# bastienjacquet/CudaDepthMapIntegration

Hardware: AMD Instinct MI355X
Metric: Gvoxel-projections/s (higher is better)
Workload: dtype f64

## Files before the change

### cudadepthmapintegration_amd/capi.py

```python
from __future__ import annotations

import ctypes
import os
import sys
from typing import NamedTuple

import numpy as np

from . import build as _build
from .scene import GridDesc, RayPotential, Views

DMI_OK = 0
DMI_F32, DMI_F64 = 0, 1
DMI_DEPTH_AUTO, DMI_DEPTH_F32, DMI_DEPTH_F64 = 0, 1, 2
DMI_COMPONENTS_MIN_TRIANGLES, DMI_COMPONENTS_LARGEST = 0, 1

VARIANT_EXACT_DIVISION = 1
VARIANT_GENERAL_K = 2
VARIANT_FORCE_GENERAL = 16
VARIANT_NO_BRICK_CLASSES = 256
VARIANT_KEEP_BEHIND_ADDS = 1024
VARIANT_NO_INTERIOR = 2048
VARIANT_XCD_RUNS = 8192
VARIANT_ZMAJOR_SLOTS = 16384
VARIANT_PERSISTENT_ALWAYS = 32768
VARIANT_PERSISTENT_NEVER = 65536
VARIANT_NO_WINDOWS = 262144
VARIANT_WINDOWS_ALWAYS = 524288
VARIANT_COST_ORDER = 1048576
VARIANT_NO_COST_ORDER = 2097152
VARIANT_BRICK_CLASSES_ALWAYS = 131072
VARIANT_FIXED_TILE_SHAPE = 4096
VARIANT_SPATIAL_ORDER = 512
VARIANT_TILE_SHAPE = {"tk16_w5_g8_1x1": 0, "tk8_w6_g8_2x2": 32, "tk16_w5_g8_2x2": 64, "tk8_w6": 96, "tk8_w7_g8": 128, "tk16_w5_g4": 160,
                      "tk16_w6_g2": 192, "tk8_w6_g8_1x1": 224}


class GridDescC(ctypes.Structure):
    _fields_ = [("cell_dims", ctypes.c_int32 * 3), ("origin", ctypes.c_double * 3),
                ("spacing", ctypes.c_double * 3), ("grid_matrix", ctypes.c_double * 16)]


class RayPotentialC(ctypes.Structure):
    _fields_ = [("thickness", ctypes.c_double), ("rho", ctypes.c_double), ("eta", ctypes.c_double),
                ("delta", ctypes.c_double)]
# ... 77 lines not shown
DMI_PARTITION_VIEWS, DMI_PARTITION_Z_SLABS = 0, 1
DMI_EXCHANGE_ALL_REDUCE, DMI_EXCHANGE_REDUCE_SCATTER, DMI_EXCHANGE_PEER_COPY = 0, 1, 2
DMI_UNIQUE_ID_BYTES = 128
RENDER_VIEW_GROUP, RENDER_LANE_CAP = 16, 64

DMI_DECIMATE_MEAN, DMI_DECIMATE_QUADRIC = 0, 1
DECIMATE_PLACEMENTS = {"mean": DMI_DECIMATE_MEAN, "quadric": DMI_DECIMATE_QUADRIC}

ABI_SYMBOLS = [
    "dmi_default_options", "dmi_create", "dmi_destroy", "dmi_last_error", "dmi_add_views", "dmi_add_views_f32",
    "dmi_clear_views", "dmi_reset_grid", "dmi_upload_grid", "dmi_fuse", "dmi_fuse_range", "dmi_fuse_slab", "dmi_fuse_range_download", "dmi_synchronize",
    "dmi_download_grid_f64", "dmi_download_grid_f32", "dmi_download_hits", "dmi_grid_device_pointer",
    "dmi_get_brick_class_histogram", "dmi_get_timings", "dmi_get_info", "dmi_alloc_pinned", "dmi_free_pinned", "dmi_pcie_probe", "dmi_fp64_probe", "dmi_abi_version", "dmi_device_count",
    "dmi_color_mesh", "dmi_color_last_error", "dmi_cell_to_point", "dmi_download_point_data_f64",
    "dmi_point_data_device_pointer", "dmi_color_create", "dmi_color_destroy", "dmi_color_add_views",
    "dmi_color_clear_views", "dmi_color_process", "dmi_color_get_kernel_ms", "dmi_get_mixed_reason_histogram", "dmi_get_window_pair_count", "dmi_get_view_paths", "dmi_get_upload_kernel_ms", "dmi_sizeof_info", "dmi_sizeof_timings",
    "dmi_color_set_scratch_budget", "dmi_color_set_vertex_reorder", "dmi_color_add_views_with_depth", "dmi_color_set_depth_test",
    "dmi_iso_active_cells",
    "dmi_extract_isosurface", "dmi_download_isosurface", "dmi_get_isosurface_kernel_ms",
    "dmi_extract_isosurface_normals", "dmi_download_isosurface_normals",
    "dmi_filter_isosurface_components", "dmi_download_isosurface_regions", "dmi_get_isosurface_filter_kernel_ms",
    "dmi_get_isosurface_filter_pass_ms", "dmi_get_isosurface_filter_cas_retries",
    "dmi_smooth_isosurface", "dmi_get_isosurface_smooth_kernel_ms", "dmi_get_isosurface_smooth_pass_ms",
    "dmi_decimate_isosurface", "dmi_get_isosurface_decimate_kernel_ms", "dmi_get_isosurface_decimate_pass_ms",
    "dmi_color_process_isosurface", "dmi_download_isosurface_colors", "dmi_get_isosurface_color_kernel_ms",
    "dmi_filter_isosurface_support", "dmi_download_isosurface_support", "dmi_get_isosurface_support_kernel_ms",
    "dmi_get_isosurface_support_pass_ms", "dmi_decimate_isosurface_placed",
    "dmi_fill_isosurface_holes", "dmi_get_isosurface_holes_kernel_ms", "dmi_get_isosurface_holes_pass_ms",
    "dmi_color_render_depths", "dmi_color_render_isosurface_depths", "dmi_color_download_depths", "dmi_color_get_render_kernel_ms",
    "dmi_color_set_render_queue_capacity", "dmi_color_get_render_pass_ms", "dmi_color_get_render_queued_pairs",
    "dmi_filter_depth_consistency", "dmi_estimate_scene_bounds", "dmi_filter_depth_speckles", "dmi_fill_depth_holes",
# ... 111 lines not shown
        L.dmi_get_isosurface_holes_pass_ms.argtypes = [vp, dp]
    if hasattr(L, "dmi_filter_isosurface_support"):
        L.dmi_filter_isosurface_support.argtypes = [vp, i32, dbl, i32, ctypes.POINTER(ctypes.c_uint64), ctypes.POINTER(ctypes.c_uint64)]
        L.dmi_download_isosurface_support.argtypes = [vp, ctypes.POINTER(ctypes.c_int32)]
        L.dmi_get_isosurface_support_kernel_ms.argtypes = [vp, dp]
        L.dmi_get_isosurface_support_pass_ms.argtypes = [vp, dp]
    if hasattr(L, "dmi_set_point_smoothing"):
        L.dmi_point_smoothing_weights.argtypes = [dbl, dbl, ctypes.POINTER(i32), dp]
        L.dmi_set_point_smoothing.argtypes = [vp, dp, dbl]
        L.dmi_get_point_smoothing.argtypes = [vp, dp, dp]
        L.dmi_get_point_smoothing_kernel_ms.argtypes = [vp, dp]
    L.dmi_get_brick_class_histogram.argtypes = [vp, ctypes.POINTER(ctypes.c_uint64)]
    L.dmi_get_mixed_reason_histogram.argtypes = [vp, ctypes.POINTER(ctypes.c_uint64)]
    if hasattr(L, "dmi_get_window_pair_count"):
        L.dmi_get_window_pair_count.argtypes = [vp, ctypes.POINTER(ctypes.c_uint64)]
    if hasattr(L, "dmi_get_view_paths"):
        L.dmi_get_view_paths.argtypes = [vp, ctypes.POINTER(ctypes.c_uint64)]
    if hasattr(L, "dmi_get_upload_kernel_ms"):
        L.dmi_get_upload_kernel_ms.argtypes = [vp, dp, dp]
    for name in ("dmi_sizeof_info", "dmi_sizeof_timings"):
        if hasattr(L, name):
            getattr(L, name).restype = ctypes.c_size_t
    L.dmi_get_timings.argtypes = [vp, ctypes.POINTER(TimingsC)]
    L.dmi_get_info.argtypes = [vp, ctypes.POINTER(InfoC)]
    L.dmi_alloc_pinned.argtypes = [ctypes.c_size_t, ctypes.POINTER(vp)]
    L.dmi_free_pinned.argtypes = [vp]
    L.dmi_pcie_probe.argtypes = [i32, ctypes.c_size_t, dp, dp]
    L.dmi_fp64_probe.argtypes = [i32, ctypes.c_double, dp]
    u8p = ctypes.POINTER(ctypes.c_uint8)
    L.dmi_color_mesh.argtypes = [dp, ctypes.c_int64, u8p, dp, dp, i32, i32, i32, i32, u8p, u8p, ctypes.POINTER(ctypes.c_int32)]
# ... 498 lines not shown

    def mixed_reason_histogram(self) -> dict:
        h = (ctypes.c_uint64 * 8)()
        self._check(self._lib.dmi_get_mixed_reason_histogram(self._h, h))
        names = ["unspecified", "degenerate", "camera_plane", "image_border", "nan_depth", "sentinel_and_depth", "near_surface",
                 "free_or_no_depth"]
        return {n: int(h[i]) for i, n in enumerate(names)}

    def window_pair_count(self) -> int:
        n = ctypes.c_uint64(0)
        if not hasattr(self._lib, "dmi_get_window_pair_count"):
            return 0
        self._check(self._lib.dmi_get_window_pair_count(self._h, ctypes.byref(n)))
        return int(n.value)

    def upload_kernel_ms(self) -> tuple:
        if not hasattr(self._lib, "dmi_get_upload_kernel_ms"):
            return (0.0, 0.0)
        a, b = ctypes.c_double(0), ctypes.c_double(0)
        self._check(self._lib.dmi_get_upload_kernel_ms(self._h, ctypes.byref(a), ctypes.byref(b)))
        return (float(a.value), float(b.value))

    def timings(self) -> TimingsC:
        t = TimingsC()
        self._check(self._lib.dmi_get_timings(self._h, ctypes.byref(t)))
        return t

    def info(self) -> InfoC:
        i = InfoC()
        self._check(self._lib.dmi_get_info(self._h, ctypes.byref(i)))
# ... 1241 lines not shown
```

### cudadepthmapintegration_amd/csrc/dmi_capi_fuse.hip

```cpp
#include "dmi_context.h"

#include <algorithm>
#include <cmath>
#include <cstdlib>
#include <cstring>

using dmi::drain_events;
using dmi::EventPair;
using dmi::fail;
using dmi::flush_zero_fill;
using dmi::FuseArgs;
using dmi::FuseConfig;
using dmi::guarded;
using dmi::MapRec;
using dmi::TileArgs;
using dmi::TileMapRec;

namespace {

static_assert(dmi::kRecordBytes[dmi::REC_MAP] == sizeof(MapRec) && dmi::kRecordBytes[dmi::REC_TILE_MAP] == sizeof(TileMapRec) &&
              dmi::kRecordBytes[dmi::REC_WIN] == sizeof(dmi::WinRec) && dmi::kRecordBytes[dmi::REC_FOOT] == sizeof(dmi::FootRec) &&
              dmi::kRecordBytes[dmi::REC_HITS] == sizeof(unsigned long long), "the record tables' rule has the records' sizes");
int sync_maps(dmi_context *ctx) {
  dmi_context::Views &v = ctx->views;
// ... 151 lines not shown
  const int rc = slot_permutation(ctx, t.super_x, t.super_y, t.super_z, (cfg.variant & dmi::VAR_ZMAJOR_SLOTS) != 0, &t.sb_perm);
  if (rc != DMI_OK) return rc;
  t.xcd_run_wg = 32 * std::max(1, t.super_x * t.super_y);
  if (((int64_t)t.super_x * t.super_y * t.super_z * 32 + 16 * (int64_t)t.xcd_run_wg + 64) > (int64_t)0x7fffffff)
    return fail(ctx, DMI_ERR_INVALID_ARGUMENT, "dmi_fuse: grid too large for one launch");
  t.depth_bytes = (int32_t)((int64_t)a.W * a.H * (ctx->views.depth_f64 ? 8 : 4));
  t.kz0 = a.kz0;
  t.ox = a.ox; t.oy = a.oy; t.oz = a.oz; t.sx = a.sx; t.sy = a.sy; t.sz = a.sz;
  std::memcpy(t.g, a.g, sizeof(t.g));
  t.thick = a.thick; t.delta = a.delta; t.rho_pos = a.rho_pos; t.rho_neg = a.rho_neg;
  t.slope = a.slope; t.free_space = a.free_space;
  t.tile_maps = ctx->views.tile_maps.as<TileMapRec>();
  t.grid = a.grid; t.voxel_hits = a.voxel_hits; t.map_hits = a.map_hits;
  t.rotated = dmi::grid_axis_aligned(ctx->grid) ? 0 : 1;
  t.flags = ((cfg.variant & dmi::VAR_NO_INTERIOR) ? dmi::TILE_FLAG_NO_INTERIOR : 0) |
            ((cfg.variant & dmi::VAR_XCD_RUNS) ? dmi::TILE_FLAG_XCD_RUNS : 0);
  t.maps = ctx->views.maps.as<MapRec>();
  t.wbricks_x = (a.nx + 7) / 8;
  t.wbricks_y = (a.ny + 7) / 8;
  return DMI_OK;
}

int cz_table(dmi_context *ctx, const FuseArgs &a, TileArgs *t) {
  const size_t table_doubles = std::max<size_t>(ctx->views.h_maps.size(), 4) * (size_t)t->kpad;
  const size_t need = table_doubles + (size_t)dmi::kFreeSumsMax + 1;
  const int rc = dmi::ensure_idle_buffer(ctx, ctx->tables.cz_table, need * 8, need * 2 * 8);
  if (rc != DMI_OK) return rc;
  t->cz_table = ctx->tables.cz_table.as<double>();
  if (!a.init_from_grid && !ctx->opt.count_hits && a.n_maps <= dmi::kFreeSumsMax) t->free_sums = t->cz_table + table_doubles;
  return DMI_OK;
}
// ... 171 lines not shown
    if (rc != DMI_OK) return rc;
    DMI_HIP(ctx, hipMemcpyAsync(ctx->tables.fuse_args.ptr, &a, sizeof(FuseArgs), hipMemcpyHostToDevice, ctx->stream));
    t.full = ctx->tables.fuse_args.as<FuseArgs>();
  }

  rc = timed_launch(ctx, a, t, cfg);
  if (rc != DMI_OK) return rc;

  dmi_context::LastLaunch &last = ctx->last;
  last.tiled = cfg.use_tile != 0;
  last.classes = cfg.use_tile != 0 && !(cfg.variant & dmi::VAR_NO_BRICK_CLASSES);
  last.class_bricks = (int64_t)t.wbricks_x * t.wbricks_y * t.bricks_z;
  last.bricks_z = t.bricks_z;
  last.tk = t.bricks_z > 0 ? t.kpad / t.bricks_z : 0;
  last.win_origin = t.win_origin;
  last.class_pitch = t.class_pitch;
  last.first = first;
  last.count = count;
  for (int32_t z = z_first; z < z_first + z_count; ++z) ctx->volume.layer_is_zero[(size_t)z] = 0;
  ctx->volume.zero_fill_pending = false;
  ctx->c2p.valid = false;
  if (ctx->pending.size() >= 256) return drain_events(ctx);
  return DMI_OK;
}

template <typename Visit>
int visit_last_classes(dmi_context *ctx, Visit &&visit) {
  const dmi_context::LastLaunch &last = ctx->last;
  if (!last.classes) return DMI_OK;
  DMI_HIP(ctx, hipSetDevice(ctx->opt.device));
// ... 90 lines not shown
int dmi_get_window_pair_count(dmi_context *ctx, uint64_t *out) {
  return guarded(ctx, "dmi_get_window_pair_count", [&]() -> int {
  if (!ctx || !out) return fail(ctx, DMI_ERR_INVALID_ARGUMENT, "dmi_get_window_pair_count: null argument");
  *out = 0;
  const dmi_context::LastLaunch &last = ctx->last;
  if (!last.win_origin) return DMI_OK;
  const int64_t per_layer = last.class_bricks / std::max<int64_t>(1, last.bricks_z);
  return visit_last_classes(ctx, [&](int64_t b, uint8_t c) {
    const int64_t bz = b / std::max<int64_t>(1, per_layer);
    if (bz * last.tk + last.tk > ctx->grid.cell_dims[2]) return;
    if ((c & 0x3f) == (dmi::BRICK_MIXED | (dmi::MIXED_FREE_OR_NODEPTH << 2))) *out += 1;
  });
  });
}

}
```

### cudadepthmapintegration_amd/csrc/dmi_context.h

```cpp
#pragma once
#include "../../include/dmi.h"
#include "dmi_buffer.h"
#include "dmi_mesh_stage.h"
#include "fusion_kernels.h"

#include <exception>
#include <initializer_list>
#include <new>
#include <string>
#include <vector>

namespace dmi {

struct Batch {
  void *d_depth = nullptr;
  DepthTile *d_pyramid = nullptr;
  size_t valid_offset = 0;
  size_t bits_offset = 0;
  size_t aux_bytes = 0;
  int32_t n = 0;
  unsigned long long holes = 0;
  unsigned long long mingled_strips = 0;
};

// ... 81 lines not shown
    std::vector<SlotPerm> slot_perms;
    dmi::DeviceBuffer order, order_level;
    void release() {
      for (SlotPerm &sp : slot_perms) dmi::free_buffers({&sp.perm});
      slot_perms.clear();
      dmi::free_buffers({&cz_table, &fuse_args, &zero_row, &classes, &queue_heads, &wg_times, &order, &order_level});
    }
  } tables;
  struct LastLaunch {
    bool tiled = false;
    bool classes = false;
    int64_t class_bricks = 0;
    int32_t bricks_z = 0, tk = 0;
    const dmi::WinPair *win_origin = nullptr;
    int32_t class_pitch = 0, first = 0, count = 0;
  } last;

  struct CellToPoint : dmi::StageTimes<2> {
    dmi::DeviceBuffer points;
    bool valid = false;
    bool pending = false;
    void release() { dmi::free_buffers({&points}); StageTimes::release(); }
  } c2p;
  struct PointSmoothing : dmi::StageTimes<2> {
    double sigma[3] = {0.0, 0.0, 0.0}, truncate = 3.0;
    bool on = false;
    dmi::PointSmoothArgs args{};
    dmi::DeviceBuffer scratch;
    bool pending = false;
    void release() { dmi::free_buffers({&scratch}); StageTimes::release(); }
// ... 131 lines not shown
```

### cudadepthmapintegration_amd/csrc/fusion_classify.hip

```cpp
#include <algorithm>
#include <cstring>

#include <stdlib.h>

#include "fusion_kernels.h"
#include "fusion_device.h"

namespace dmi {

namespace {

template <typename T>
__device__ __forceinline__ T cload(const T *p) {
  return *reinterpret_cast<const T __attribute__((address_space(4))) *>(reinterpret_cast<uintptr_t>(p));
}

__device__ __forceinline__ float float_below(double d) {
  float f = (float)d;
  if ((double)f > d) f = nextafterf(f, -__builtin_inff());
  return f;
}
__device__ __forceinline__ float float_above(double d) {
  float f = (float)d;
  if ((double)f < d) f = nextafterf(f, __builtin_inff());
// ... 362 lines not shown
  if (c == BRICK_SKIP || (c == BRICK_BEHIND && a.behind_mask)) return BRICK_SKIP;
  const bool map_serves = DMI_TIER1 != 0 && !GK && fp.in_margin && a.behind_mask != 0;
  if (map_serves && (c == BRICK_FREE || c == (uint8_t)(BRICK_MIXED | (MIXED_FREE_OR_NODEPTH << 2))))
    return BRICK_MIXED | (MIXED_FREE_OR_NODEPTH << 2);
  return BRICK_MIXED | (MIXED_IMAGE_BORDER << 2);
}

template <int kQueryTiles, bool ROT, bool GK>
__device__ __forceinline__ uint8_t classify_box(const TileArgs &a, const MapRec *__restrict__ mr,
                                                const TileMapRec *__restrict__ tr, const PyramidDesc &P, int i0, int i1,
                                                int j0, int j1, int k0, int k1) {
  const BoxFootprint fp = box_footprint<ROT, GK>(a, mr, tr, i0, i1, j0, j1, k0, k1);
  if (fp.partial) return border_class<GK>(a, fp, pyramid_query<kQueryTiles>(mr->pyramid, P, fp.x0, fp.x1, fp.y0, fp.y1));
  if (!fp.query) return fp.cls;
  return class_from_bounds(a, pyramid_query<kQueryTiles>(mr->pyramid, P, fp.x0, fp.x1, fp.y0, fp.y1), fp.czmin, fp.czmax);
}

constexpr int kCostLevels = 64;

template <bool ROT, bool GK>
__global__ __launch_bounds__(256) void classify_coarse_kernel(const TileArgs a, const MapRec *__restrict__ maps,
                                                              const PyramidDesc P, int tk, uint8_t *__restrict__ classes,
                                                              uint8_t *__restrict__ coarse) {
  fill_launch_tables(a, maps, ((int64_t)blockIdx.y * gridDim.x + blockIdx.x) * 256 + threadIdx.y * 64 + threadIdx.x,
                     (int64_t)gridDim.x * gridDim.y * 256);
  if ((a.flags & TILE_FLAG_COST_ORDER) && blockIdx.x == 0 && blockIdx.y == 0 && threadIdx.y == 0)
    for (int q = threadIdx.x; q < 2 * kCostLevels; q += 64) const_cast<int32_t *>(a.order_levels)[q] = 0;
  const int bz_first = 2 * a.sbz_first;
  const int bz_count = min(2 * a.super_z, a.bricks_z - bz_first);
  const int per_z = 32 / tk;
// ... 68 lines not shown
  while (items) {
    const int first = __builtin_ctzll(items);
    items &= items - 1;
    const int rel = first + lane / children;
    const int mm = chunk0 + rel;
    const int m = a.first_map + min(mm, a.n_maps - 1);
    const bool mine = in_grid && ((unproven >> rel) & 1ull);
    const MapRec *__restrict__ mr = maps + m;
    BoxFootprint fp;
    fp.query = false;
    fp.partial = false;
    fp.in_margin = false;
    fp.cls = BRICK_SKIP;
    MapRec mr_u;
    TileMapRec tr_u;
    if constexpr (views_per_wave == 1) {
      const int mu = __builtin_amdgcn_readfirstlane(m);
      const MapRec *src = maps + mu;
      const TileMapRec *tsrc = a.tile_maps + mu;
#pragma unroll
      for (int q = 8; q < 12; ++q) mr_u.rt[q] = cload(&src->rt[q]);
      mr_u.pyramid = cload(&src->pyramid);
      tr_u.px = cload(&tsrc->px); tr_u.py = cload(&tsrc->py); tr_u.pz = cload(&tsrc->pz); tr_u.p0 = cload(&tsrc->p0);
      tr_u.qx = cload(&tsrc->qx); tr_u.qy = cload(&tsrc->qy); tr_u.qz = cload(&tsrc->qz); tr_u.q0 = cload(&tsrc->q0);
      tr_u.err = cload(&tsrc->err);
      tr_u.cz_err = cload(&tsrc->cz_err);
      tr_u.errz = cload(&tsrc->errz);
      if constexpr (GK) {
        tr_u.sx = cload(&tsrc->sx); tr_u.sy = cload(&tsrc->sy); tr_u.sz = cload(&tsrc->sz); tr_u.s0 = cload(&tsrc->s0);
      }
      mr = &mr_u;
      if (mine) {
        fp = box_footprint<ROT, GK>(a, &mr_u, &tr_u, bx * 8, bx * 8 + 7, by * 8, by * 8 + 7, bz * tk, bz * tk + tk - 1);
      }
    } else {
      if (mine) fp = box_footprint<ROT, GK>(a, mr, a.tile_maps + m, bx * 8, bx * 8 + 7, by * 8, by * 8 + 7, bz * tk, bz * tk + tk - 1);
    }
    const bool query = mine && (fp.query || fp.partial);
    uint8_t cls = fp.cls;
    const int li = query ? query_level<kQueryTiles>(P, max(fp.x1 - fp.x0, fp.y1 - fp.y0) + 1) : 0x7fff;
    bool from_window = false;
    {
      float2 *__restrict__ win_mm = window_mm[wave * views_per_wave + lane / children];
      uint8_t *__restrict__ win_fl = window_fl[wave * views_per_wave + lane / children];
      int li_w = li;
      for (int off = children >> 1; off > 0; off >>= 1) li_w = min(li_w, __shfl_xor(li_w, off, 64));
      if (li_w != 0x7fff) {
        const int L = kPyramidMinLevel + li_w;
        const bool at_level = query && li == li_w;
        int tx0 = at_level ? fp.x0 >> L : 0x7fffffff, ty0 = at_level ? fp.y0 >> L : 0x7fffffff;
        int tx1 = at_level ? fp.x1 >> L : -1, ty1 = at_level ? fp.y1 >> L : -1;
        int wx0 = tx0, wy0 = ty0, wx1 = tx1, wy1 = ty1;
        for (int off = children >> 1; off > 0; off >>= 1) {
          wx0 = min(wx0, __shfl_xor(wx0, off, 64));
          wy0 = min(wy0, __shfl_xor(wy0, off, 64));
          wx1 = max(wx1, __shfl_xor(wx1, off, 64));
// ... 10 lines not shown
              win_mm[ty * kWindow + tx] = make_float2(t.dmin, t.dmax);
              win_fl[ty * kWindow + tx] = (uint8_t)t.flags;
            }
          __builtin_amdgcn_fence(__ATOMIC_RELEASE, "wavefront");
          __builtin_amdgcn_wave_barrier();
          __builtin_amdgcn_fence(__ATOMIC_ACQUIRE, "wavefront");
          if (at_level) {
            TileAcc d;
            for (int ty = ty0; ty <= ty1; ++ty)
              for (int tx = tx0; tx <= tx1; ++tx) {
                const int w = (ty - wy0) * kWindow + (tx - wx0);
                const float2 mm = win_mm[w];
                d.add_tile(DepthTile{mm.x, mm.y, (uint32_t)win_fl[w], 0u});
              }
            cls = fp.partial ? border_class<GK>(a, fp, d) : class_from_bounds(a, d, fp.czmin, fp.czmax);
            from_window = true;
          }
          __builtin_amdgcn_fence(__ATOMIC_RELEASE, "wavefront");
          __builtin_amdgcn_wave_barrier();
        }
      }
    }
    if (query && !from_window) {
      const TileAcc d = pyramid_query<kQueryTiles>(mr->pyramid, P, fp.x0, fp.x1, fp.y0, fp.y1);
      cls = fp.partial ? border_class<GK>(a, fp, d) : class_from_bounds(a, d, fp.czmin, fp.czmax);
    }
    if (mine) out[m] = cls;
  }
}

constexpr int kOriginViews = 8;
#ifdef DMI_WINPAIR_BRICK_MAJOR
constexpr int kOriginBricks = 256, kOriginWaveSets = 1, kOriginAlign = 4;
#else
constexpr int kOriginBricks = 64, kOriginWaveSets = 4, kOriginAlign = kWinPairBlockViews;
static_assert(kOriginViews * kOriginWaveSets == kWinPairBlockViews, "a workgroup's views are one block of the pair table");
#endif
constexpr uint32_t kNotWanted = 0xfffffffeu;
template <bool ROT>
__global__ __launch_bounds__(256) void window_origin_kernel(const TileArgs a, const MapRec *__restrict__ maps, int tk,
                                                            uint8_t *__restrict__ classes, WinPair *__restrict__ origins,
                                                            int group_views) {
// ... 570 lines not shown
```

### cudadepthmapintegration_amd/csrc/fusion_kernels.h

```cpp
#pragma once

#include <hip/hip_runtime.h>
#include <stddef.h>
#include <stdint.h>
#include <string.h>

#include "fusion_launch_rules.h"
#include "point_smooth_rules.h"
#include "view_records.h"

struct dmi_context;

namespace dmi {

int grid_pointer_for_sums(::dmi_context *ctx, void **ptr);

struct alignas(16) DepthTile {
  float dmin, dmax;
  uint32_t flags;
  uint32_t pad;
};
enum TileFlags : uint32_t { TILE_HAS_SENTINEL = 1, TILE_HAS_VALID = 2, TILE_HAS_NAN = 4, TILE_PART_HOLE_FREE = 8, TILE_PART_NO_VALID = 16 };
constexpr uint8_t COARSE_CHILDREN_WRITTEN = 0x80;

// ... 5 lines not shown
  int32_t total_tiles;
  int32_t width[kPyramidMaxLevels];
  int32_t height[kPyramidMaxLevels];
  int32_t offset[kPyramidMaxLevels];
};

#ifndef DMI_TIER1
#define DMI_TIER1 1
#endif
constexpr uint8_t CLASS_NO_WINDOW = 0x20;
struct alignas(16) WinPair {
  uint32_t origin;
  float ax, ay, acz;
};
static_assert(sizeof(WinPair) == 16, "WinPair layout");

struct FuseArgs {
  int32_t nx, ny, nz;
  int32_t W, H;
  int32_t first_map, n_maps;
  int32_t init_from_grid;
  int32_t kz0, pad1;
  int32_t k_first, k_count;
  double ox, oy, oz;
  double sx, sy, sz;
  double g[12];
  double thick, delta;
  double rho_pos, rho_neg, rho_zero;
  double slope;
  double free_space;
// ... 41 lines not shown
  int64_t n_class_bricks;
  const WinRec *win_recs;
  const FootRec *foot_recs;
  int32_t vb_bytes, vb_rowskip;
  int32_t win_cx, win_cy;
};
constexpr int kFreeSumsMax = 4096;
__host__ __device__ inline int32_t pack_brick(int bx, int by, int bz) { return (int32_t)((uint32_t)bx | ((uint32_t)by << 11) | ((uint32_t)bz << 22)); }
static_assert(offsetof(TileArgs, nx) == 0 && offsetof(TileArgs, nz) == 8 && offsetof(TileArgs, kpad) == 32 &&
                  offsetof(TileArgs, bricks_x) == 36 && offsetof(TileArgs, bricks_z) == 44 && offsetof(TileArgs, sbz_first) == 60,
              "TileArgs head layout");
enum TileKernelFlags : int32_t {
  TILE_FLAG_NO_INTERIOR = 1,
  TILE_FLAG_XCD_RUNS = 2,
  TILE_FLAG_COST_ORDER = 4,
  TILE_FLAG_DBG_SKIP_WINDOW_PAIRS = 256,
  TILE_FLAG_DBG_ONLY_WINDOW_PAIRS = 512,
  TILE_FLAG_DBG_NO_WINDOW_LOADS = 1024
};

enum BrickClass : uint8_t {
  BRICK_MIXED = 0,
  BRICK_FREE = 1,
  BRICK_BEHIND = 2,
  BRICK_SKIP = 3
};

enum MixedReason : uint8_t {
  MIXED_UNSPECIFIED = 0,
  MIXED_DEGENERATE = 1,
// ... 220 lines not shown
```

### cudadepthmapintegration_amd/csrc/fusion_launch_rules.h

```cpp
#pragma once
#include <stddef.h>
#include <stdint.h>

namespace dmi {

constexpr int64_t kNoClassesMaxBricks = 1024;
constexpr int kNoClassesMaxViews = 48;

enum VariantBits : int {
  VAR_EXACT_DIVISION = 1,
  VAR_GENERAL_K = 2,
  VAR_BLOCK_SHAPE_MASK = 12,
  VAR_FORCE_GENERAL = 16,
  VAR_TILE_SHAPE_MASK = 0xE0,
  VAR_TILE_SHAPE_SHIFT = 5,
  VAR_NO_BRICK_CLASSES = 256,
  VAR_SPATIAL_ORDER = 512,
  VAR_FIXED_TILE_SHAPE = 4096,
  VAR_KEEP_BEHIND_ADDS = 1024,
  VAR_NO_INTERIOR = 2048,
  VAR_XCD_RUNS = 8192,
  VAR_ZMAJOR_SLOTS = 16384,
  VAR_PERSISTENT_ALWAYS = 32768,
  VAR_PERSISTENT_NEVER = 65536,
  VAR_BRICK_CLASSES_ALWAYS = 131072,
  VAR_NO_WINDOWS = 262144,
  VAR_WINDOWS_ALWAYS = 524288,
  VAR_COST_ORDER = 1048576,
  VAR_NO_COST_ORDER = 2097152
};

constexpr int kCostOrderMaxSlots = 0;

struct HoleTraits {
  bool scattered = false;
  bool holes = false;
  bool tall_by_holes = false;
  bool many_borders = false;
  bool mostly_empty = false;
};

inline HoleTraits hole_traits(unsigned long long mingled, unsigned long long without, unsigned long long strips, unsigned long long pixels) {
  HoleTraits h;
  h.scattered = without <= 6 * mingled;
  h.holes = h.scattered && mingled * 160 > strips;
// ... 84 lines not shown
```

### cudadepthmapintegration_amd/csrc/fusion_tile.hip

```cpp
#include <stdlib.h>

#include <algorithm>
#include <type_traits>

#include "fusion_kernels.h"
#include "fusion_device.h"

#ifndef DMI_T1_CHAINS
#define DMI_T1_CHAINS 4
#endif
#ifndef DMI_T1_COLUMN_CHAINS
#define DMI_T1_COLUMN_CHAINS 2
#endif
#if !defined(DMI_TUNING) && (defined(DMI_EXP_SKIP_WINDOW_VIEWS) || defined(DMI_EXP_SAME_REC) || defined(DMI_EXP_NO_WINDOW_LOADS) || \
                             defined(DMI_EXP_NO_LANE_MARGIN))
#error "a DMI_EXP_* switch that changes results was defined without DMI_TUNING"
#endif

namespace dmi {

int tile_shape_index(int variant);

namespace {

// ... 953 lines not shown
      }
    }

    [[maybe_unused]] auto rot_cz = [&](int kk) __attribute__((always_inline)) -> double {
      if (kk >= kcount) return -__builtin_inf();
      const kernarg_t kr = KFRESH();
      const TileMapRec *rr = kr->tile_maps + m;
      const czvec4 b = cload(reinterpret_cast<const czvec4 *>(kr->cz_table + (int64_t)(k0 + kk) * 4));
      const double wxk = (wx + b[0]) + kr->g[3], wyk = (wy + b[1]) + kr->g[7], wzk = (wz0 + b[2]) + kr->g[11];
      return ((cload(&rr->rz0) * wxk + cload(&rr->rz1) * wyk) + cload(&kr->maps[m].rt[10]) * wzk) + sz;
    };

    uint32_t undecided = 0;
    uint32_t und_kk = 0;
    uint32_t map_hits = 0;

    auto column = [&](auto interior_tag, auto surface_tag, auto free_tag) __attribute__((always_inline)) {
      constexpr bool INTERIOR = decltype(interior_tag)::value;
      constexpr bool FREEONLY = decltype(free_tag)::value;
      constexpr bool SURFACE = decltype(surface_tag)::value;
      constexpr bool UNMASKED = INTERIOR && !COUNT;
      [[maybe_unused]] int cxc = 0, cyc = 0;
      [[maybe_unused]] unsigned bias_x = 0, bias_y = 0;
      if constexpr (T1 && !INTERIOR) {
        cxc = KC(W) >> 1;
        cyc = KC(H) >> 1;
        bias_x = 0x4B400000u - (unsigned)cxc;
        bias_y = 0x4B400000u - (unsigned)cyc;
        if constexpr (kConstantsInVgprs) asm volatile("" : "+v"(bias_x), "+v"(bias_y));
      }
      constexpr bool VMAP = T1 && FREEONLY;
      const __amdgpu_buffer_rsrc_t rsrc =
          __builtin_amdgcn_make_buffer_rsrc(const_cast<void *>(cload(&rec->depth)), (short)0, KC(depth_bytes), 0x00020000);
      mask_t m_lane_ok = m_lane_ok_brick;
      asm volatile("" : "+s"(m_lane_ok));
      [[maybe_unused]] __amdgpu_buffer_rsrc_t vrsrc = rsrc;
      [[maybe_unused]] float v_c0 = 0.f, v_w8 = 0.f;
      [[maybe_unused]] int v_base = 0;
      if constexpr (VMAP) {
        vrsrc = __builtin_amdgcn_make_buffer_rsrc(const_cast<uint8_t *>(cload(&rec->valid)), (short)0, cload(&rec->vm_bytes), 0x00020000);
        v_c0 = cload(&rec->vm_c0);
        v_w8 = cload(&rec->vm_w8);
        v_base = cload(&rec->vm_base);
      }
  #pragma unroll
      for (int g0 = 0; g0 < TK; g0 += kGroup) {
        double czg[kGroup];
        typename DL::raw_t dg[kGroup];
        [[maybe_unused]] unsigned short vg[kGroup];
        if constexpr (!ROT && !(T1 && FREEONLY)) {
          const czvec ctg = cload(reinterpret_cast<const czvec *>(ct + g0));
  #pragma unroll
          for (int q = 0; q < kGroup; ++q) czg[q] = (sz + ctg[q]) + rz3;
          __builtin_amdgcn_sched_barrier(0);
        }
        if constexpr (ROT && T1 && !FREEONLY) {
          const double c20 = cload(&rec->rz0), c21 = cload(&rec->rz1), c22 = cload(&kv->maps[m].rt[10]);
  #pragma unroll
          for (int q = 0; q < kGroup; ++q) {
            const int kk = g0 + q;
            czg[q] = -__builtin_inf();
// ... 96 lines not shown
              }
              m_und &= ~m_p2;
            }
            if constexpr (VMAP && UNMASKED) {
              vg[q] = __builtin_amdgcn_raw_buffer_load_b8(vrsrc, (int)pix, 0, 0);
              if (m_und) {
                or_where(undecided, m_und, 1u << kk);
                und_kk |= 1u << kk;
                if (__builtin_amdgcn_inverse_ballot_w64(m_und)) vg[q] = 0;
              }
            } else if constexpr (UNMASKED) {
              dg[q] = DL::load_at(rsrc, pix);
              if (m_und) {
                or_where(undecided, m_und, 1u << kk);
                und_kk |= 1u << kk;
                if (__builtin_amdgcn_inverse_ballot_w64(m_und)) dg[q] = SURFACE ? DL::minus_inf() : DL::sentinel();
              }
            } else {
              if (m_und) {
                or_where(undecided, m_und, 1u << kk);
                und_kk |= 1u << kk;
              }
              if (__builtin_amdgcn_inverse_ballot_w64(m_in)) dg[q] = DL::load_at(rsrc, pix);
            }
            continue;
          }
          if constexpr (ROT) {
            if (kk >= kcount) continue;
            const czvec4 b = cload(reinterpret_cast<const czvec4 *>(kv->cz_table + (int64_t)(k0 + kk) * 4));
            const double wxk = (wx + b[0]) + KA(g)[3], wyk = (wy + b[1]) + KA(g)[7], wzk = (wz0 + b[2]) + KA(g)[11];
            czg[q] = ((r20 * wxk + r21 * wyk) + r22 * wzk) + sz;
// ... 52 lines not shown
            }
          } else {
            const int px = cvt_saturating(ru), py = cvt_saturating(rv);
            if constexpr (!INTERIOR)
              m_in &= ballot((unsigned)px < vW) & ballot((unsigned)py < vH);
            if (m_und) {
              or_where(undecided, m_und, 1u << kk);
              und_kk |= 1u << kk;
            }
            if (__builtin_amdgcn_inverse_ballot_w64(m_in))
              dg[q] = DL::load(rsrc, __umul24((unsigned)py, vW) + (unsigned)px);
          }
        }
        }
  #pragma unroll
        for (int q = 0; q < kGroup; ++q) {
          const int kk = g0 + q;
          if constexpr (VMAP) {
            static_assert(kValidByte == 10, "((1 << 10) - 1) << 20 == 0x3ff00000");
            unsigned one_or_zero_hi;
            asm("v_bfm_b32 %0, %1, 20" : "=v"(one_or_zero_hi) : "v"(__builtin_bit_cast(_Float16, vg[q])));
            acc_fma_vs<BASE, TK>(kk, __hiloint2double((int)one_or_zero_hi, 0), free_space);
            continue;
          }
          const typename DL::raw_t d = dg[q];
          if constexpr (ZF && !FREEONLY) {
            if constexpr (std::is_same<DepthT, double>::value) {
              if constexpr (SURFACE) acc_potential_all_f64<BASE, TK>(kk, d, czg[q], delta, thick, slope, free_space, rho_pos);
              else acc_potential_f64<BASE, TK>(kk, d, czg[q], delta, thick, slope, free_space, rho_pos);
            } else {
              if constexpr (SURFACE) acc_potential_all_f32<BASE, TK>(kk, d, czg[q], delta, thick, slope, free_space, rho_pos);
// ... 14 lines not shown
            if (!SURFACE && keep_zero_adds) acc_add_zero<BASE, TK>(kk, m_hit & m_behind_far);
            const mask_t m_near = m_hit & ~(m_front_far | m_behind_far);
            {
              if (m_near) {
                const int rh = __double2hiint(rho_pos) ^ (__double2hiint(diff) & (int)0x80000000);
                const double near = __builtin_fabs(diff) > thick ? __hiloint2double(rh, __double2loint(rho_pos)) : slope * diff;
                acc_add_v<BASE, TK>(kk, m_near, near);
              }
            }
            if (COUNT) {
              nh[kk] += __builtin_amdgcn_inverse_ballot_w64(m_hit) ? 1u : 0u;
              map_hits += (uint32_t)__popcll(m_hit);
            }
          }
        }
      }
    };
    const bool interior = kcount == TK && (cbyte & 0x1fu) >= ((unsigned)MIXED_NAN_DEPTH << 2) && !(kv->flags & TILE_FLAG_NO_INTERIOR);
    if (interior) {
      if constexpr (!COUNT) {
        if ((cbyte & 0x1fu) == ((unsigned)MIXED_FREE_OR_NODEPTH << 2 | BRICK_MIXED))
          column(std::true_type{}, std::false_type{}, std::true_type{});
#ifndef DMI_EXP_NO_SURFACE_COLUMN
        else if ((cbyte & 0x1fu) == ((unsigned)MIXED_NEAR_SURFACE << 2 | BRICK_MIXED) && !keep_zero_adds)
          column(std::true_type{}, std::true_type{}, std::false_type{});
#endif
        else
          column(std::true_type{}, std::false_type{}, std::false_type{});
      } else {
        column(std::true_type{}, std::false_type{}, std::false_type{});
      }
    } else {
      column(std::false_type{}, std::false_type{}, std::false_type{});
// ... 296 lines not shown
```

### include/dmi.h

```cpp
#ifndef DMI_H_
#define DMI_H_

#include <stddef.h>
#include <stdint.h>

#ifdef __cplusplus
extern "C" {
#endif

#define DMI_ABI_VERSION 5

typedef struct dmi_context dmi_context;

typedef enum dmi_status {
  DMI_OK = 0,
  DMI_ERR_INVALID_ARGUMENT = 1,
  DMI_ERR_DEVICE = 2,
  DMI_ERR_OUT_OF_MEMORY = 3,
  DMI_ERR_STATE = 4
} dmi_status;

typedef enum dmi_dtype { DMI_F32 = 0, DMI_F64 = 1 } dmi_dtype;

typedef enum dmi_depth_storage { DMI_DEPTH_AUTO = 0, DMI_DEPTH_F32 = 1, DMI_DEPTH_F64 = 2 } dmi_depth_storage;
// ... 359 lines not shown
int dmi_multi_clear_views(dmi_multi_context *ctx);

int dmi_multi_fuse(dmi_multi_context *ctx);
int dmi_multi_synchronize(dmi_multi_context *ctx);

int dmi_multi_download_grid_f32(dmi_multi_context *ctx, float *out, int64_t *owned_first, int64_t *owned_count);
int dmi_multi_download_grid_f64(dmi_multi_context *ctx, double *out, int64_t *owned_first, int64_t *owned_count);

int dmi_multi_get_info(dmi_multi_context *ctx, dmi_multi_info *out);
int dmi_multi_get_timings(dmi_multi_context *ctx, dmi_multi_timings *out);
int dmi_multi_local_context(dmi_multi_context *ctx, int32_t local_index, dmi_context **out);

int dmi_abi_version(void);
int dmi_device_count(void);

#ifdef __cplusplus
}
#endif

#endif
```

Baseline: 3193.

## Classify near-surface bricks per 4-layer group to skip behind and front layers

```diff
diff --git a/cudadepthmapintegration_amd/capi.py b/cudadepthmapintegration_amd/capi.py
--- a/cudadepthmapintegration_amd/capi.py
+++ b/cudadepthmapintegration_amd/capi.py
@@ -29,6 +29,7 @@
 VARIANT_WINDOWS_ALWAYS = 524288
 VARIANT_COST_ORDER = 1048576
 VARIANT_NO_COST_ORDER = 2097152
+VARIANT_NO_LAYER_GROUP_CLASSES = 4194304
 VARIANT_BRICK_CLASSES_ALWAYS = 131072
 VARIANT_FIXED_TILE_SHAPE = 4096
 VARIANT_SPATIAL_ORDER = 512
@@ -136,7 +137,7 @@
     "dmi_get_brick_class_histogram", "dmi_get_timings", "dmi_get_info", "dmi_alloc_pinned", "dmi_free_pinned", "dmi_pcie_probe", "dmi_fp64_probe", "dmi_abi_version", "dmi_device_count",
     "dmi_color_mesh", "dmi_color_last_error", "dmi_cell_to_point", "dmi_download_point_data_f64",
     "dmi_point_data_device_pointer", "dmi_color_create", "dmi_color_destroy", "dmi_color_add_views",
-    "dmi_color_clear_views", "dmi_color_process", "dmi_color_get_kernel_ms", "dmi_get_mixed_reason_histogram", "dmi_get_window_pair_count", "dmi_get_view_paths", "dmi_get_upload_kernel_ms", "dmi_sizeof_info", "dmi_sizeof_timings",
+    "dmi_color_clear_views", "dmi_color_process", "dmi_color_get_kernel_ms", "dmi_get_mixed_reason_histogram", "dmi_get_window_pair_count", "dmi_get_layer_group_counts", "dmi_get_view_paths", "dmi_get_upload_kernel_ms", "dmi_sizeof_info", "dmi_sizeof_timings",
     "dmi_color_set_scratch_budget", "dmi_color_set_vertex_reorder", "dmi_color_add_views_with_depth", "dmi_color_set_depth_test",
     "dmi_iso_active_cells",
     "dmi_extract_isosurface", "dmi_download_isosurface", "dmi_get_isosurface_kernel_ms",
@@ -278,6 +279,8 @@
     L.dmi_get_mixed_reason_histogram.argtypes = [vp, ctypes.POINTER(ctypes.c_uint64)]
     if hasattr(L, "dmi_get_window_pair_count"):
         L.dmi_get_window_pair_count.argtypes = [vp, ctypes.POINTER(ctypes.c_uint64)]
+    if hasattr(L, "dmi_get_layer_group_counts"):
+        L.dmi_get_layer_group_counts.argtypes = [vp, ctypes.POINTER(ctypes.c_uint64)]
     if hasattr(L, "dmi_get_view_paths"):
         L.dmi_get_view_paths.argtypes = [vp, ctypes.POINTER(ctypes.c_uint64)]
     if hasattr(L, "dmi_get_upload_kernel_ms"):
@@ -806,6 +809,12 @@
         self._check(self._lib.dmi_get_window_pair_count(self._h, ctypes.byref(n)))
         return int(n.value)
 
+    def layer_group_counts(self) -> dict:
+        h = (ctypes.c_uint64 * 4)()
+        if hasattr(self._lib, "dmi_get_layer_group_counts"):
+            self._check(self._lib.dmi_get_layer_group_counts(self._h, h))
+        return {"pairs": int(h[0]), "groups": int(h[1]), "behind": int(h[2]), "front": int(h[3])}
+
     def upload_kernel_ms(self) -> tuple:
         if not hasattr(self._lib, "dmi_get_upload_kernel_ms"):
             return (0.0, 0.0)
diff --git a/cudadepthmapintegration_amd/csrc/dmi_capi_fuse.hip b/cudadepthmapintegration_amd/csrc/dmi_capi_fuse.hip
--- a/cudadepthmapintegration_amd/csrc/dmi_capi_fuse.hip
+++ b/cudadepthmapintegration_amd/csrc/dmi_capi_fuse.hip
@@ -189,7 +189,8 @@
   t.grid = a.grid; t.voxel_hits = a.voxel_hits; t.map_hits = a.map_hits;
   t.rotated = dmi::grid_axis_aligned(ctx->grid) ? 0 : 1;
   t.flags = ((cfg.variant & dmi::VAR_NO_INTERIOR) ? dmi::TILE_FLAG_NO_INTERIOR : 0) |
-            ((cfg.variant & dmi::VAR_XCD_RUNS) ? dmi::TILE_FLAG_XCD_RUNS : 0);
+            ((cfg.variant & dmi::VAR_XCD_RUNS) ? dmi::TILE_FLAG_XCD_RUNS : 0) |
+            ((cfg.variant & dmi::VAR_NO_LAYER_GROUP_CLASSES) ? dmi::TILE_FLAG_NO_LAYER_GROUPS : 0);
   t.maps = ctx->views.maps.as<MapRec>();
   t.wbricks_x = (a.nx + 7) / 8;
   t.wbricks_y = (a.ny + 7) / 8;
@@ -391,6 +392,7 @@
   last.bricks_z = t.bricks_z;
   last.tk = t.bricks_z > 0 ? t.kpad / t.bricks_z : 0;
   last.win_origin = t.win_origin;
+  last.layer_groups = dmi::kLayerGroupClasses && t.win_origin != nullptr && t.behind_mask != 0 && !cfg.general_k && !(t.flags & dmi::TILE_FLAG_NO_LAYER_GROUPS);
   last.class_pitch = t.class_pitch;
   last.first = first;
   last.count = count;
@@ -511,4 +513,36 @@
   });
 }
 
-}
+int dmi_get_layer_group_counts(dmi_context *ctx, uint64_t out[4]) {
+  return guarded(ctx, "dmi_get_layer_group_counts", [&]() -> int {
+  if (!ctx || !out) return fail(ctx, DMI_ERR_INVALID_ARGUMENT, "dmi_get_layer_group_counts: null argument");
+  out[0] = out[1] = out[2] = out[3] = 0;
+  const dmi_context::LastLaunch &last = ctx->last;
+  if (!last.classes || !last.layer_groups || last.tk <= 0) return DMI_OK;
+  DMI_HIP(ctx, hipSetDevice(ctx->opt.device));
+  const size_t entries = (size_t)last.class_bricks * last.class_pitch;
+  std::vector<uint8_t> classes(entries);
+  std::vector<dmi::LayerGroupPair> pairs(entries);
+  DMI_HIP(ctx, hipMemcpyAsync(classes.data(), ctx->tables.classes.ptr, entries, hipMemcpyDeviceToHost, ctx->stream));
+  DMI_HIP(ctx, hipMemcpyAsync(pairs.data(), last.win_origin, entries * sizeof(dmi::LayerGroupPair), hipMemcpyDeviceToHost, ctx->stream));
+  DMI_HIP(ctx, hipStreamSynchronize(ctx->stream));
+  const int64_t per_layer = last.class_bricks / std::max<int64_t>(1, last.bricks_z);
+  const int groups = last.tk / dmi::kLayerGroup;
+  const uint32_t group_bits = (1u << groups) - 1u;
+  for (int64_t b = 0; b < last.class_bricks; ++b) {
+    if ((b / std::max<int64_t>(1, per_layer)) * last.tk + last.tk > ctx->grid.cell_dims[2]) continue;
+    for (int32_t m = last.first; m < last.first + last.count; ++m) {
+      const uint8_t c = classes[(size_t)b * last.class_pitch + m] & 0x1f;
+      if (c != (dmi::BRICK_MIXED | (dmi::MIXED_NEAR_SURFACE << 2)) && c != (dmi::BRICK_MIXED | (dmi::MIXED_SENTINEL_AND_DEPTH << 2))) continue;
+      const uint32_t w = pairs[(size_t)dmi::win_pair_index(b, m, last.class_bricks)].masks;
+      out[0] += 1;
+      out[1] += (uint64_t)groups;
+      out[2] += (uint64_t)__builtin_popcount(w & group_bits);
+      out[3] += (uint64_t)__builtin_popcount((w >> dmi::kLayerGroupFrontShift) & group_bits);
+    }
+  }
+  return DMI_OK;
+  });
+}
+
+}
diff --git a/cudadepthmapintegration_amd/csrc/dmi_context.h b/cudadepthmapintegration_amd/csrc/dmi_context.h
--- a/cudadepthmapintegration_amd/csrc/dmi_context.h
+++ b/cudadepthmapintegration_amd/csrc/dmi_context.h
@@ -119,6 +119,7 @@
     int32_t bricks_z = 0, tk = 0;
     const dmi::WinPair *win_origin = nullptr;
     int32_t class_pitch = 0, first = 0, count = 0;
+    bool layer_groups = false;
   } last;
 
   struct CellToPoint : dmi::StageTimes<2> {
diff --git a/cudadepthmapintegration_amd/csrc/fusion_classify.hip b/cudadepthmapintegration_amd/csrc/fusion_classify.hip
--- a/cudadepthmapintegration_amd/csrc/fusion_classify.hip
+++ b/cudadepthmapintegration_amd/csrc/fusion_classify.hip
@@ -400,6 +400,21 @@
   if (fp.partial) return border_class<GK>(a, fp, pyramid_query<kQueryTiles>(mr->pyramid, P, fp.x0, fp.x1, fp.y0, fp.y1));
   if (!fp.query) return fp.cls;
   return class_from_bounds(a, pyramid_query<kQueryTiles>(mr->pyramid, P, fp.x0, fp.x1, fp.y0, fp.y1), fp.czmin, fp.czmax);
+}
+
+template <int TK, bool ROT>
+__device__ __forceinline__ uint32_t layer_group_masks(const TileArgs &a, const MapRec *__restrict__ mr, const TileMapRec *__restrict__ tr,
+                                                      const TileAcc &d, int i0, int i1, int j0, int j1, int k0) {
+  uint32_t word = 0;
+#pragma unroll
+  for (int g = 0; g < TK / kLayerGroup; ++g) {
+    const BoxFootprint s = box_footprint_k<ROT, false>(a, mr, tr, i0, i1, j0, j1, k0 + kLayerGroup * g, k0 + kLayerGroup * g + kLayerGroup - 1);
+    if ((s.czmin - (double)d.dmax) > a.delta)
+      word |= 1u << g;
+    else if ((s.czmax - (double)d.dmin) < -a.delta)
+      word |= 1u << (kLayerGroupFrontShift + g);
+  }
+  return word;
 }
 
 constexpr int kCostLevels = 64;
@@ -498,6 +513,7 @@
     fp.cls = BRICK_SKIP;
     MapRec mr_u;
     TileMapRec tr_u;
+    const TileMapRec *__restrict__ tr = a.tile_maps + m;
     if constexpr (views_per_wave == 1) {
       const int mu = __builtin_amdgcn_readfirstlane(m);
       const MapRec *src = maps + mu;
@@ -514,16 +530,18 @@
         tr_u.sx = cload(&tsrc->sx); tr_u.sy = cload(&tsrc->sy); tr_u.sz = cload(&tsrc->sz); tr_u.s0 = cload(&tsrc->s0);
       }
       mr = &mr_u;
+      tr = &tr_u;
       if (mine) {
         fp = box_footprint<ROT, GK>(a, &mr_u, &tr_u, bx * 8, bx * 8 + 7, by * 8, by * 8 + 7, bz * tk, bz * tk + tk - 1);
       }
     } else {
-      if (mine) fp = box_footprint<ROT, GK>(a, mr, a.tile_maps + m, bx * 8, bx * 8 + 7, by * 8, by * 8 + 7, bz * tk, bz * tk + tk - 1);
+      if (mine) fp = box_footprint<ROT, GK>(a, mr, tr, bx * 8, bx * 8 + 7, by * 8, by * 8 + 7, bz * tk, bz * tk + tk - 1);
     }
     const bool query = mine && (fp.query || fp.partial);
     uint8_t cls = fp.cls;
     const int li = query ? query_level<kQueryTiles>(P, max(fp.x1 - fp.x0, fp.y1 - fp.y0) + 1) : 0x7fff;
     bool from_window = false;
+    TileAcc dq;
     {
       float2 *__restrict__ win_mm = window_mm[wave * views_per_wave + lane / children];
       uint8_t *__restrict__ win_fl = window_fl[wave * views_per_wave + lane / children];
@@ -564,6 +582,7 @@
                 d.add_tile(DepthTile{mm.x, mm.y, (uint32_t)win_fl[w], 0u});
               }
             cls = fp.partial ? border_class<GK>(a, fp, d) : class_from_bounds(a, d, fp.czmin, fp.czmax);
+            dq = d;
             from_window = true;
           }
           __builtin_amdgcn_fence(__ATOMIC_RELEASE, "wavefront");
@@ -574,8 +593,21 @@
     if (query && !from_window) {
       const TileAcc d = pyramid_query<kQueryTiles>(mr->pyramid, P, fp.x0, fp.x1, fp.y0, fp.y1);
       cls = fp.partial ? border_class<GK>(a, fp, d) : class_from_bounds(a, d, fp.czmin, fp.czmax);
+      dq = d;
     }
     if (mine) out[m] = cls;
+    if constexpr (kLayerGroupClasses && !GK) {
+      if (a.win_origin != nullptr && a.behind_mask != 0 && !(a.flags & TILE_FLAG_NO_LAYER_GROUPS)) {
+        const uint8_t reason = cls & 0x1f;
+        if (mine && (reason == (uint8_t)(BRICK_MIXED | (MIXED_NEAR_SURFACE << 2)) || reason == (uint8_t)(BRICK_MIXED | (MIXED_SENTINEL_AND_DEPTH << 2)))) {
+          constexpr int kTK = 512 / kChildren;
+          LayerGroupPair e{0u, {0u, 0u, 0u}};
+          if (fp.query && bz * kTK + kTK <= a.nz) e.masks = layer_group_masks<kTK, ROT>(a, mr, tr, dq, bx * 8, bx * 8 + 7, by * 8, by * 8 + 7, bz * kTK);
+          const int64_t brick = ((int64_t)bz * a.wbricks_y + by) * a.wbricks_x + bx;
+          reinterpret_cast<LayerGroupPair *>(a.win_origin)[win_pair_index(brick, m, a.n_class_bricks)] = e;
+        }
+      }
+    }
   }
 }
 
diff --git a/cudadepthmapintegration_amd/csrc/fusion_kernels.h b/cudadepthmapintegration_amd/csrc/fusion_kernels.h
--- a/cudadepthmapintegration_amd/csrc/fusion_kernels.h
+++ b/cudadepthmapintegration_amd/csrc/fusion_kernels.h
@@ -43,6 +43,18 @@
   float ax, ay, acz;
 };
 static_assert(sizeof(WinPair) == 16, "WinPair layout");
+struct alignas(16) LayerGroupPair {
+  uint32_t masks;
+  uint32_t unused[3];
+};
+static_assert(sizeof(LayerGroupPair) == sizeof(WinPair) && offsetof(LayerGroupPair, masks) == offsetof(WinPair, origin),
+              "a layer-group entry takes a window pair's slot, its word where the origin is");
+static_assert(kMaxLayerGroups <= kLayerGroupFrontShift && 2 * kLayerGroupFrontShift <= 32, "both masks of the tallest column in one word");
+#if defined(DMI_NO_LAYER_GROUP_CLASSES) || defined(DMI_WINPAIR_LANE_HELD) || defined(DMI_WINPAIR_BRICK_MAJOR)
+constexpr bool kLayerGroupClasses = false;
+#else
+constexpr bool kLayerGroupClasses = true;
+#endif
 
 struct FuseArgs {
   int32_t nx, ny, nz;
@@ -114,6 +126,7 @@
   TILE_FLAG_NO_INTERIOR = 1,
   TILE_FLAG_XCD_RUNS = 2,
   TILE_FLAG_COST_ORDER = 4,
+  TILE_FLAG_NO_LAYER_GROUPS = 8,
   TILE_FLAG_DBG_SKIP_WINDOW_PAIRS = 256,
   TILE_FLAG_DBG_ONLY_WINDOW_PAIRS = 512,
   TILE_FLAG_DBG_NO_WINDOW_LOADS = 1024
diff --git a/cudadepthmapintegration_amd/csrc/fusion_launch_rules.h b/cudadepthmapintegration_amd/csrc/fusion_launch_rules.h
--- a/cudadepthmapintegration_amd/csrc/fusion_launch_rules.h
+++ b/cudadepthmapintegration_amd/csrc/fusion_launch_rules.h
@@ -27,8 +27,13 @@
   VAR_NO_WINDOWS = 262144,
   VAR_WINDOWS_ALWAYS = 524288,
   VAR_COST_ORDER = 1048576,
-  VAR_NO_COST_ORDER = 2097152
+  VAR_NO_COST_ORDER = 2097152,
+  VAR_NO_LAYER_GROUP_CLASSES = 4194304
 };
+
+constexpr int kLayerGroup = 4;
+constexpr int kMaxLayerGroups = 16 / kLayerGroup;
+constexpr int kLayerGroupFrontShift = 8;
 
 constexpr int kCostOrderMaxSlots = 0;
 
diff --git a/cudadepthmapintegration_amd/csrc/fusion_tile.hip b/cudadepthmapintegration_amd/csrc/fusion_tile.hip
--- a/cudadepthmapintegration_amd/csrc/fusion_tile.hip
+++ b/cudadepthmapintegration_amd/csrc/fusion_tile.hip
@@ -991,12 +991,19 @@
     uint32_t undecided = 0;
     uint32_t und_kk = 0;
     uint32_t map_hits = 0;
+    [[maybe_unused]] uint32_t lg_masks = 0;
+    constexpr bool kLayerGroups = kLayerGroupClasses && WIN && ZF && T1;
 
     auto column = [&](auto interior_tag, auto surface_tag, auto free_tag) __attribute__((always_inline)) {
       constexpr bool INTERIOR = decltype(interior_tag)::value;
       constexpr bool FREEONLY = decltype(free_tag)::value;
       constexpr bool SURFACE = decltype(surface_tag)::value;
       constexpr bool UNMASKED = INTERIOR && !COUNT;
+      constexpr bool LG = kLayerGroups && INTERIOR && !FREEONLY && !COUNT;
+      constexpr int kSub = LG ? kLayerGroup : kGroup;
+      static_assert(kGroup % kSub == 0 && TK % kSub == 0, "whole layer groups per load group");
+      [[maybe_unused]] auto lg_behind = [&](int kk) __attribute__((always_inline)) { return ((lg_masks >> (kk / kLayerGroup)) & 1u) != 0; };
+      [[maybe_unused]] auto lg_front = [&](int kk) __attribute__((always_inline)) { return ((lg_masks >> (kLayerGroupFrontShift + kk / kLayerGroup)) & 1u) != 0; };
       [[maybe_unused]] int cxc = 0, cyc = 0;
       [[maybe_unused]] unsigned bias_x = 0, bias_y = 0;
       if constexpr (T1 && !INTERIOR) {
@@ -1022,6 +1029,10 @@
       }
   #pragma unroll
       for (int g0 = 0; g0 < TK; g0 += kGroup) {
+        if constexpr (LG) {
+          constexpr uint32_t halves = (1u << (kGroup / kLayerGroup)) - 1u;
+          if (((lg_masks >> (g0 / kLayerGroup)) & halves) == halves) continue;
+        }
         double czg[kGroup];
         typename DL::raw_t dg[kGroup];
         [[maybe_unused]] unsigned short vg[kGroup];
@@ -1148,7 +1159,9 @@
               if (m_und) {
                 or_where(undecided, m_und, 1u << kk);
                 und_kk |= 1u << kk;
-                if (__builtin_amdgcn_inverse_ballot_w64(m_und)) dg[q] = SURFACE ? DL::minus_inf() : DL::sentinel();
+                bool as_no_depth = !SURFACE;
+                if constexpr (LG && SURFACE) as_no_depth = lg_front(kk);
+                if (__builtin_amdgcn_inverse_ballot_w64(m_und)) dg[q] = as_no_depth ? DL::sentinel() : DL::minus_inf();
               }
             } else {
               if (m_und) {
@@ -1231,7 +1244,17 @@
         }
         }
   #pragma unroll
-        for (int q = 0; q < kGroup; ++q) {
+        for (int s0 = 0; s0 < kGroup; s0 += kSub) {
+        if constexpr (LG) {
+          if (lg_behind(g0 + s0)) continue;
+          if (lg_front(g0 + s0)) {
+  #pragma unroll
+            for (int q = s0; q < s0 + kSub; ++q) acc_add_s<BASE, TK>(g0 + q, ballot(!DL::is_sentinel(dg[q])), free_space);
+            continue;
+          }
+        }
+  #pragma unroll
+        for (int q = s0; q < s0 + kSub; ++q) {
           const int kk = g0 + q;
           if constexpr (VMAP) {
             static_assert(kValidByte == 10, "((1 << 10) - 1) << 20 == 0x3ff00000");
@@ -1276,9 +1299,18 @@
             }
           }
         }
+        }
       }
     };
     const bool interior = kcount == TK && (cbyte & 0x1fu) >= ((unsigned)MIXED_NAN_DEPTH << 2) && !(kv->flags & TILE_FLAG_NO_INTERIOR);
+    if constexpr (kLayerGroups) {
+      const unsigned reason = cbyte & 0x1fu;
+      const bool near_surface = reason == ((unsigned)MIXED_NEAR_SURFACE << 2 | BRICK_MIXED) || reason == ((unsigned)MIXED_SENTINEL_AND_DEPTH << 2 | BRICK_MIXED);
+      if (interior && near_surface && !(kv->flags & TILE_FLAG_NO_LAYER_GROUPS)) {
+        pair_area_wait();
+        lg_masks = (uint32_t)__builtin_amdgcn_readfirstlane((int)pair_area()[m & (kPairGroupViews - 1)].x);
+      }
+    }
     if (interior) {
       if constexpr (!COUNT) {
         if ((cbyte & 0x1fu) == ((unsigned)MIXED_FREE_OR_NODEPTH << 2 | BRICK_MIXED))
diff --git a/include/dmi.h b/include/dmi.h
--- a/include/dmi.h
+++ b/include/dmi.h
@@ -397,6 +397,8 @@
 int dmi_abi_version(void);
 int dmi_device_count(void);
 
+int dmi_get_layer_group_counts(dmi_context *ctx, uint64_t out[4]);
+
 #ifdef __cplusplus
 }
 #endif
```

After: 3074. 3.7% lower.
